# ayushpradhan-dev/robust-speech-analysis-framework

Measured on AMD Instinct MI355X. Metric: audio-seconds processed/sec (extract+CNN-LSTM fwd), higher is better.
Workload: dtype f32

## Files before the change

robust_speech_analysis_framework_amd/csrc/mshds_pitch.hip:

```cpp
#include <algorithm>
#include <map>
#include <mutex>
#include <vector>

#include "mshds_common.h"
#include "mshds_pitch_layout.h"

namespace rsaf {
namespace mshds {

struct PitchParams {
    double dt, min_pitch, ceiling, voicing_thr, octave_cost, dt_window;
    int cheb_all_full;
    int cheb_clipped;
    int nsamp_window, half_window, nsamp_period, half_period, min_lag, max_lag, brent_ixmax, max_cand;
    int refine_depth, is_cc;
    int nfft;
    double voicing_thr2;
    int debug_stop;
};

struct FrameOut {
    double intensity;
    double ncand;
// ... 593 lines not shown
            if (l0 + 1 <= L) {
                const double den = sumx2 * yb[m];
                rb[l0 + 1] = (l0 + 1 <= loc_max_lag && den > 0.0) ? (-y[m].y * inv_n) * fast_rsqrt(den) : 0.0;
            }
        }
        wave_sync();
    }
}

constexpr int CT = 64;
struct DeferArgs {
    FrameHdr* hdr;
    double* pc_a;
    double* pc_b;
    int grouped;
};
struct CandCtx {
    const PitchParams& P;
    const DeferArgs& DA;
    const double* cheb;
    int lane;
    int L, RC, RN;
    int nz_lo, nz_hi;
    double* r;
    double *s_mfreq, *s_mstr, *s_mloc;
    int* s_maxlag;
    int* s_cnt;
    double* s_part;
};

// ... 137 lines not shown
    const bool cand_lane = lane >= 1 && lane < nc;
    const int my_b0 = (cand_lane ? place_lag[lane] : 0) + RC - 1;
    if (use_cheb && !P.cheb_all_full) {
        int dc0 = P.refine_depth, dc1 = P.refine_depth;
        dc0 = dc0 < my_b0 + 1 ? dc0 : my_b0 + 1;
        dc0 = dc0 < RN - my_b0 - 1 ? dc0 : RN - my_b0 - 1;
        dc1 = dc1 < my_b0 + 2 ? dc1 : my_b0 + 2;
        dc1 = dc1 < RN - my_b0 - 2 ? dc1 : RN - my_b0 - 2;
        n_clip_cols = __popcll(__ballot(cand_lane && dc0 < P.refine_depth)) + __popcll(__ballot(cand_lane && dc1 < P.refine_depth));
        const int dmin = cand_row_min(cand_lane ? min(dc0, dc1) : P.refine_depth);
        if (n_clip_cols > 0 && (!P.cheb_clipped || dmin < 3)) use_cheb = false;
    }
    return CandClip{use_cheb, n_clip_cols, cand_lane, my_b0};
}

__device__ __forceinline__ void cand_coef_4x4x4(const CandCtx& X, int nc, const int* place_lag, const CandClip& C) {
    const double* cheb = X.cheb;
    const int lane = X.lane, RC = X.RC, nz_lo = X.nz_lo, nz_hi = X.nz_hi;
    const double* r = X.r;
    const bool cand_lane = C.cand_lane;
    const int my_b0 = C.my_b0;
    double* s_P = X.s_part;
    const int d = X.P.refine_depth;
    const int kq = lane >> 4, nn = lane & 15;
    const int ncol = 2 * (nc - 1);
    const int bmin = cand_row_min(cand_lane ? my_b0 : 0x7fffffff), bmax = -cand_row_min(cand_lane ? -my_b0 : 0x7fffffff);
    const int groups = (ncol + 3) >> 2;
    int rb4[3];
    bool cf4[3];
#pragma unroll
    for (int g = 0; g < 3; ++g) {
        const int n = 4 * g + (lane & 3), k = 1 + (n >> 1);
        rb4[g] = place_lag[k < nc ? k : 1] + RC - 1 + (n & 1);
        cf4[g] = n < ncol;
    }
    int o_lo = nz_lo - (bmax + 1), o_hi = nz_hi - bmin;
    o_lo = o_lo < -(d - 1) ? -(d - 1) : o_lo;
    o_hi = o_hi > d ? d : o_hi;
    double a4[3] = {0.0, 0.0, 0.0};
    const double* ctab = cheb + (int64_t)(d - 1) * NCH + nn;
    int o = o_lo;
    for (; o + 31 <= o_hi; o += 32) {
        double cw[8];
#pragma unroll
        for (int u = 0; u < 8; ++u) cw[u] = ctab[(int64_t)(o + 4 * u + kq) * NCH];
#pragma unroll
        for (int u = 0; u < 8; ++u) {
            const int oo = o + 4 * u + kq;
            a4[0] = __builtin_amdgcn_mfma_f64_4x4x4f64(cw[u], cf4[0] ? r[rb4[0] + oo] : 0.0, a4[0], 0, 0, 0);
            if (groups > 1) a4[1] = __builtin_amdgcn_mfma_f64_4x4x4f64(cw[u], cf4[1] ? r[rb4[1] + oo] : 0.0, a4[1], 0, 0, 0);
            if (groups > 2) a4[2] = __builtin_amdgcn_mfma_f64_4x4x4f64(cw[u], cf4[2] ? r[rb4[2] + oo] : 0.0, a4[2], 0, 0, 0);
        }
    }
    for (; o <= o_hi; o += 4) {
        const int oo = o + kq, oc = oo <= o_hi ? oo : o_hi;
        const double cw = oo <= o_hi ? ctab[(int64_t)oc * NCH] : 0.0;
        a4[0] = __builtin_amdgcn_mfma_f64_4x4x4f64(cw, cf4[0] ? r[rb4[0] + oc] : 0.0, a4[0], 0, 0, 0);
        if (groups > 1) a4[1] = __builtin_amdgcn_mfma_f64_4x4x4f64(cw, cf4[1] ? r[rb4[1] + oc] : 0.0, a4[1], 0, 0, 0);
        if (groups > 2) a4[2] = __builtin_amdgcn_mfma_f64_4x4x4f64(cw, cf4[2] ? r[rb4[2] + oc] : 0.0, a4[2], 0, 0, 0);
    }
    const int coef = (nn & 12) + kq;
#pragma unroll
    for (int g = 0; g < 3; ++g) {
        const int n = 4 * g + (lane & 3), k = 1 + (n >> 1);
        if (g < groups && n < ncol) s_P[(k * 2 + (n & 1)) * NCH + coef] = a4[g];
    }
}

__device__ __forceinline__ void cand_coef_16x16x4(const CandCtx& X, int nc, const int* place_lag, const CandClip& C) {
    const double* cheb = X.cheb;
    const int lane = X.lane, RC = X.RC, RN = X.RN, nz_lo = X.nz_lo, nz_hi = X.nz_hi;
    const double* r = X.r;
    const bool cand_lane = C.cand_lane;
    const int my_b0 = C.my_b0, n_clip_cols = C.n_clip_cols;
    double* s_P = X.s_part;
    const int d = X.P.refine_depth;
    const int kq = lane >> 4, nn = lane & 15;
    const int ncol = 2 * (nc - 1), tiles = (ncol + 15) >> 4;
    const int bmin = cand_row_min(cand_lane ? my_b0 : 0x7fffffff), bmax = -cand_row_min(cand_lane ? -my_b0 : 0x7fffffff);
    int rbase[2];
    bool colfull[2];
#pragma unroll
    for (int T = 0; T < 2; ++T) {
        const int n = 16 * T + nn, k = 1 + (n >> 1);
        rbase[T] = place_lag[k < nc ? k : 1] + RC - 1 + (n & 1);
        colfull[T] = n_clip_cols == 0 || (rbase[T] + 1 >= d && RN - rbase[T] - 1 >= d);
    }
    int o_lo = nz_lo - (bmax + 1), o_hi = nz_hi - bmin;
    o_lo = o_lo < -(d - 1) ? -(d - 1) : o_lo;
    o_hi = o_hi > d ? d : o_hi;
    double4_t acc0 = {0.0, 0.0, 0.0, 0.0}, acc1 = acc0;
    const double* ctab = cheb + (int64_t)(d - 1) * NCH + nn;
    int o = o_lo;
    for (; o + 31 <= o_hi; o += 32) {
        double cw[8];
#pragma unroll
        for (int u = 0; u < 8; ++u) cw[u] = ctab[(int64_t)(o + 4 * u + kq) * NCH];
#pragma unroll
        for (int u = 0; u < 8; ++u) {
            const int oo = o + 4 * u + kq;
            acc0 = __builtin_amdgcn_mfma_f64_16x16x4f64(cw[u], colfull[0] ? r[rbase[0] + oo] : 0.0, acc0, 0, 0, 0);
            if (tiles > 1) acc1 = __builtin_amdgcn_mfma_f64_16x16x4f64(cw[u], colfull[1] ? r[rbase[1] + oo] : 0.0, acc1, 0, 0, 0);
        }
    }
    for (; o <= o_hi; o += 4) {
        const int oo = o + kq, oc = oo <= o_hi ? oo : o_hi;
        const double cw = oo <= o_hi ? ctab[(int64_t)oc * NCH] : 0.0;
        acc0 = __builtin_amdgcn_mfma_f64_16x16x4f64(cw, colfull[0] ? r[rbase[0] + oc] : 0.0, acc0, 0, 0, 0);
        if (tiles > 1) acc1 = __builtin_amdgcn_mfma_f64_16x16x4f64(cw, colfull[1] ? r[rbase[1] + oc] : 0.0, acc1, 0, 0, 0);
    }
#pragma unroll
    for (int T = 0; T < 2; ++T) {
        const int n = 16 * T + nn, k = 1 + (n >> 1);
        if (T < tiles && k < nc) {
#pragma unroll
            for (int v = 0; v < 4; ++v) s_P[(k * 2 + (n & 1)) * NCH + kq + 4 * v] = T == 0 ? acc0[v] : acc1[v];
        }
    }
}

__device__ __forceinline__ void cand_coef_clipped_cells(const CandCtx& X, int nc, const int* place_lag) {
    const double* cheb = X.cheb;
    const int lane = X.lane, RC = X.RC, RN = X.RN;
    const double* r = X.r;
    double* s_P = X.s_part;
    const int d = X.P.refine_depth;
    const int ncol = 2 * (nc - 1);
    __builtin_amdgcn_fence(__ATOMIC_RELEASE, "workgroup");
    __builtin_amdgcn_wave_barrier();
    __builtin_amdgcn_fence(__ATOMIC_ACQUIRE, "workgroup");
    const double* clip_tabs = cheb + (int64_t)2 * d * NCH;
    const int jj = lane & 15, ph = lane >> 4;
    for (int col = 0; col < ncol; ++col) {
        const int k = 1 + (col >> 1), b = place_lag[k] + RC - 1 + (col & 1);
        int dc = d;
        dc = dc < b + 1 ? dc : b + 1;
        dc = dc < RN - b - 1 ? dc : RN - b - 1;
        if (dc >= d) continue;
        const double* tab = clip_tabs + (int64_t)NCH * dc * (dc - 1) + jj;
        double acc = 0.0;
        int o = -(dc - 1) + ph;
        for (; o + 12 <= dc; o += 16) {
            double tw4[4];
#pragma unroll
            for (int u = 0; u < 4; ++u) tw4[u] = tab[(int64_t)(o + 4 * u + dc - 1) * NCH];
#pragma unroll
            for (int u = 0; u < 4; ++u) acc = fma(tw4[u], r[b + o + 4 * u], acc);
        }
        for (; o <= dc; o += 4) acc = fma(tab[(int64_t)(o + dc - 1) * NCH], r[b + o], acc);
        acc += __shfl_xor(acc, 16, 64);
        acc += __shfl_xor(acc, 32, 64);
        if (ph == 0) s_P[(k * 2 + (col & 1)) * NCH + jj] = acc;
    }
}

__device__ __forceinline__ bool cand_hand_over_or_brent(const CandCtx& X, int nc, const int* place_lag, double* cf, double* cs,
                                                        double* pc_out) {
    const DeferArgs& DA = X.DA;
    const int tid = X.lane, RC = X.RC;
    const double* s_P = X.s_part;
    if (DA.hdr) {
        for (int i = 2 * NCH + tid; i < nc * 2 * NCH; i += CT) pc_out[i] = s_P[i];
        __syncthreads();
        return true;
    }
    if (tid < 64) {
        const int k = 1 + tid;
// ... 12 lines not shown
const int tid = X.lane, L = X.L, RC = X.RC, RN = X.RN, nz_lo = X.nz_lo, nz_hi = X.nz_hi;
const double* r = X.r;
    const int nref = nc - 1;
    const int span = P.refine_depth < 2 * L ? P.refine_depth : 2 * L;
    RefineArgs A{r, RN, RC, P.refine_depth, nz_lo, nz_hi, nc, place_lag, cf, cs};
    if (nref <= 4) { if (span >= 6 * 64) refine_candidates<64, true>(A, tid, CT); else refine_candidates<64, false>(A, tid, CT); }
    else if (nref <= 8) { if (span >= 6 * 32) refine_candidates<32, true>(A, tid, CT); else refine_candidates<32, false>(A, tid, CT); }
    else { if (span >= 6 * 16) refine_candidates<16, true>(A, tid, CT); else refine_candidates<16, false>(A, tid, CT); }
    __syncthreads();
}

__device__ __forceinline__ bool cand_refine_list(const CandCtx& X, int nc, const int* place_lag, double* cf, double* cs,
                                                 double* pc_out) {
    if (X.DA.hdr && X.DA.grouped) return true;
    const CandClip C = cand_clip_analysis(X, nc, place_lag);
    if (C.use_cheb) {
        const int ncol = 2 * (nc - 1);
        if (nc > 1 && ncol <= 12 && C.n_clip_cols == 0) {
            cand_coef_4x4x4(X, nc, place_lag, C);
        } else if (nc > 1) {
            cand_coef_16x16x4(X, nc, place_lag, C);
            if (C.n_clip_cols > 0) cand_coef_clipped_cells(X, nc, place_lag);
        }
        __syncthreads();
        if (X.P.debug_stop == 6) return true;
        return cand_hand_over_or_brent(X, nc, place_lag, cf, cs, pc_out);
    }
    cand_refine_direct(X, nc, place_lag, cf, cs);
    return false;
}

__device__ __forceinline__ void cand_write_hdr(FrameHdr* hdr, int tid, int flags, int n_a, const int* pl_a, int n_b,
                                               const int* pl_b, int hit) {
    if (tid < MAXC) {
        hdr->lag_a[tid] = (uint16_t)pl_a[tid];
        if (pl_b) {
            hdr->lag_b[tid] = (uint16_t)pl_b[tid];
// ... 18 lines not shown

__global__ __launch_bounds__(64) void pitch_cand_kernel(const ClipInfo* __restrict__ ci, const double* __restrict__ gpeak,
                                                        const PitchParams P, const double* __restrict__ rbuf, int rstride,
                                                        int max_frames, FrameOut* __restrict__ out,
                                                        FrameOut* __restrict__ out2, const double* __restrict__ cheb,
                                                        const DeferArgs DA) {
    extern __shared__ __attribute__((aligned(16))) char smem_raw[];
    const ClipInfo c = ci[blockIdx.y];
    const int f = blockIdx.x;
    if (f >= c.n_frames) return;
    const int tid = threadIdx.x, lane = tid & 63;
    const int L = P.is_cc ? P.max_lag : P.brent_ixmax;
    const int RC = P.brent_ixmax;
    const int RN = 2 * P.brent_ixmax + 1;
    int r_lo, r_hi;
    pitch_r_range(RC, L, P.min_lag, P.max_lag, (DA.hdr && DA.grouped) ? 30 : P.refine_depth, &r_lo, &r_hi);
    const CandLds lds(r_lo, r_hi);
    double* r_store = lds.r_store(smem_raw);
    double* r = r_store - (RC + r_lo);
    double* lists = lds.lists(smem_raw);
    int* ilists = reinterpret_cast<int*>(lists);
    double* s_mfreq = lists + CandLds::MFREQ;
    double* s_mstr = lists + CandLds::MSTR;
    double* s_mloc = lists + CandLds::MLOC;
    double* s_cf = lists + CandLds::CF;
    double* s_cs = lists + CandLds::CS;
    double* s_cloc = lists + CandLds::CLOC;
    int* s_maxlag = ilists + CandLds::MAXLAG;
    int* s_place = ilists + CandLds::PLACE;
    int* s_place2 = ilists + CandLds::PLACE2;
    int* s_cnt = ilists + CandLds::CNT;
// ... 182 lines not shown
        if (m1) qb[count + __popcll(b1 & below)] = ((unsigned)g << 5) | ((unsigned)m1 << 1) | 1u;
        count += __popcll(b1);
        wave_sync();
        int done = 0;
        for (; count - done >= 16; done += 16) run_tile(done, 16);
        const int left = count - done;
        const unsigned rest = lane < left ? qb[done + lane] : 0u;
        wave_sync();
        if (lane < left) qb[lane] = rest;
        count = left;
        wave_sync();
    }
    if (count > 0) run_tile(0, count);
}

__global__ __launch_bounds__(64) void pitch_brent_kernel(const ClipInfo* __restrict__ ci, const int* __restrict__ hdr,
                                                         const double* __restrict__ pc_a, const double* __restrict__ pc_b,
                                                         int max_frames, int RC, FrameOut* __restrict__ out_a,
                                                         FrameOut* __restrict__ out_b) {
    const ClipInfo c = ci[blockIdx.y];
    const int f0 = blockIdx.x * BR_FRAMES;
    if (f0 >= c.n_frames) return;
    const int lane = threadIdx.x;
    const int64_t g0 = (int64_t)blockIdx.y * max_frames + f0;
    int cnt_a = 0, cnt_b = 0;
    if (lane < BR_FRAMES && f0 + lane < c.n_frames) {
        const FrameHdr* h = FrameHdr::at(hdr, g0 + lane);
        const int flags = h->flags;
        if (flags & HDR_A_DEFER) cnt_a = h->n_a > 1 ? h->n_a - 1 : 0;
        if (flags & HDR_B_DEFER) cnt_b = h->n_b > 1 ? h->n_b - 1 : 0;
// ... 305 lines not shown
    FrameOut* frame_out;
    unsigned char* psi;
    int* end_state;
    double *sel_freq, *sel_strength, *stats;
    bool complete() const { return frame_out && psi && end_state && sel_freq && sel_strength && stats; }
};

struct PitchPlan {
    PitchParams P;
    double silence_thr, octave_jump, vuv;
    bool dual;
    int seg_len, Lr, rstride;
    int ncc, log2m, log2n;
    int wave_r;
    size_t lds_corr, lds_cand, lds_cell;
    int cell_b_lo, cell_n_b, cell_ntap_pad;
    bool defer;
    bool grouped;
    const double* cheb;
    int group;
    double corr_flops, corr_lds;
};

static int64_t cell_workgroups(const PitchPlan& pl, int64_t gframes, int* n_chunks_out) {
    const int64_t n_chunks = (gframes + CELL_CHUNK_FRAMES - 1) / CELL_CHUNK_FRAMES;
    if (n_chunks_out) *n_chunks_out = (int)n_chunks;
    return 8 * (int64_t)pl.cell_n_b * ((n_chunks + 7) / 8);
}

static int pitch_plan(const PitchCall& c, const double* h, const PitchOutputs& o1, const PitchOutputs& o2,
                      double voicing_thr2, PitchPlan* plan) {
    PitchPlan& pl = *plan;
    PitchParams& P = pl.P;
// ... 22 lines not shown
    RSAF_CHECK_ARG((P.is_cc ? P.max_lag : P.brent_ixmax) <= 1023, "more than 1023 lags (pitch floor below ~16 Hz) is not supported");
    P.nfft = 1;
    while ((double)P.nfft < (double)P.nsamp_window * 1.5) P.nfft *= 2;
    if (P.nfft < 16) P.nfft = 16;
    RSAF_CHECK_ARG(P.is_cc || P.nsamp_window + P.brent_ixmax <= P.nfft, "brent_ixmax must not exceed half the analysis window");
    const int seg_len = pl.seg_len = P.is_cc ? P.nsamp_window + P.max_lag + 1 : P.nsamp_window;
    const int Lr = pl.Lr = pitch_row_lags(h);
    pl.rstride = Lr + 2;
    int ncc = 64;
    while (ncc < seg_len) ncc *= 2;
    RSAF_CHECK_ARG(!P.is_cc || ncc <= 4096, "cross-correlation window + lag range longer than 4 095 samples is not supported");
    RSAF_CHECK_ARG(P.is_cc || P.nfft <= 4096, "autocorrelation window longer than 2 730 samples is not supported");
    pl.lds_corr = P.is_cc ? CcLds(ncc, Lr).bytes() : 0;
    pl.defer = getenv("RSAF_PITCH_INKERNEL") == nullptr;
    pl.grouped = pl.defer && table_mode == 2 && !dual && P.is_cc && c.sinc_cheb != nullptr;
    int r_lo_h, r_hi_h;
    pitch_r_range(P.brent_ixmax, Lr, P.min_lag, P.max_lag, pl.grouped ? 30 : P.refine_depth, &r_lo_h, &r_hi_h);
    pl.lds_cand = CandLds(r_lo_h, r_hi_h).bytes();
    RSAF_CHECK_ARG(pl.lds_corr <= 150 * 1024 && pl.lds_cand <= 150 * 1024, "analysis window too long for LDS");
    const int64_t row_bytes_per_clip = (int64_t)max_frames * PitchWs::bytes_per_frame(pl.rstride);
    RSAF_CHECK_ARG(max_frames == 0 || (c.workspace && c.workspace_bytes >= row_bytes_per_clip),
                   "workspace too small (rsaf_mshds_pitch_workspace_bytes)");
    int group = max_frames == 0 ? n_clips : (int)std::min<int64_t>(n_clips, c.workspace_bytes / std::max<int64_t>(row_bytes_per_clip, 1));
    if (max_frames > 0) group = (int)std::min<int64_t>(group, ((int64_t)1 << 26) / max_frames > 0 ? ((int64_t)1 << 26) / max_frames : 1);
    pl.group = group;
    RSAF_CHECK_ARG(table_mode != 2 || (!dual && P.is_cc), "per-cell tables serve single-threshold cross-correlation analyses only");
    pl.log2m = 0;
    while ((2 << pl.log2m) < P.nfft) ++pl.log2m;
    pl.log2n = 0;
    while ((1 << pl.log2n) < ncc) ++pl.log2n;
    int wave_r = 0;
    if (!P.is_cc) wave_r = pl.log2m <= 9 ? 8 : 1 << (pl.log2m - 6);
    else if (pl.log2n <= 11) wave_r = pl.log2n <= 10 ? 16 : 32;
    if (wave_r && !P.is_cc) P.nfft = 128 * wave_r;
    if (wave_r && P.is_cc) ncc = 64 * wave_r;
    pl.wave_r = wave_r;
    pl.ncc = ncc;
    pl.cheb = table_mode == 2 ? nullptr : c.sinc_cheb;
    const int cell_lag_lo = P.min_lag > 2 ? P.min_lag : 2;
    const int cell_lag_hi = std::min(P.max_lag - 1, P.brent_ixmax - 1);
    const bool unclipped = P.brent_ixmax + cell_lag_lo - 1 >= P.refine_depth && cell_lag_hi + 2 + P.refine_depth <= P.brent_ixmax;
    P.cheb_all_full = unclipped ? 1 : 0;
    if (pl.cheb == nullptr) P.cheb_clipped = 0;
    if (!unclipped && !P.cheb_clipped) pl.cheb = nullptr;
    pl.cell_b_lo = P.brent_ixmax + cell_lag_lo - 1;
    pl.cell_n_b = cell_lag_hi - cell_lag_lo + 2;
    pl.cell_ntap_pad = (Lr + 1 + 3) & ~3;
    pl.lds_cell = CellLds(pl.cell_ntap_pad).bytes();
    if (pl.grouped) {
        RSAF_CHECK_ARG(pl.cell_n_b >= 1 && pl.lds_cell <= 150 * 1024, "per-cell tables: lag range too long for LDS");
        if (max_frames > 0 && P.debug_stop == 0)
            RSAF_CHECK_ARG(cell_workgroups(pl, (int64_t)group * max_frames, nullptr) <= 0x7fffffffLL,
                           "per-cell tables: too many workgroups");
    }
    const double Mfft = 0.5 * (double)P.nfft;
    const double ac_flops = 2.0 * 5.0 * Mfft * log2(Mfft) + 30.0 * Mfft;
    const double cc_flops = 5.0 * ncc * log2((double)ncc) + 2.5 * ncc * log2(0.5 * ncc) + 40.0 * 0.5 * ncc + 4.0 * seg_len;
    const double ac_lds = 160.0 * Mfft;
    const double cc_lds = wave_r ? 120.0 * ncc + 16.0 * Lr
// ... 6 lines not shown
static int pitch_prepare(const PitchPlan& pl, const double2_t** tw_out, const double2_t** tw2_out) {
    if (!pl.wave_r)
        RSAF_CHECK_HIP(hipFuncSetAttribute((const void*)pitch_cc_kernel<12>, hipFuncAttributeMaxDynamicSharedMemorySize, (int)pl.lds_corr));
    const double *tw = nullptr, *tw2 = nullptr;
    int rc = fft_twiddles(pl.P.is_cc ? 2 * pl.ncc : pl.P.nfft, &tw);
    if (rc == RSAF_OK && pl.P.is_cc) rc = fft_twiddles(pl.ncc, &tw2);
    if (rc != RSAF_OK) return rc;
    *tw_out = reinterpret_cast<const double2_t*>(tw);
    *tw2_out = reinterpret_cast<const double2_t*>(tw2);
    if (pl.lds_cand > 48 * 1024)
        RSAF_CHECK_HIP(hipFuncSetAttribute((const void*)pitch_cand_kernel, hipFuncAttributeMaxDynamicSharedMemorySize,
                                           (int)pl.lds_cand));
    if (pl.grouped && pl.lds_cell > 48 * 1024)
        RSAF_CHECK_HIP(hipFuncSetAttribute((const void*)pitch_cell_coef_kernel, hipFuncAttributeMaxDynamicSharedMemorySize,
                                           (int)pl.lds_cell));
    return RSAF_OK;
}

struct PitchGroup {
    const ClipInfo* ci;
    const double* gpeak;
    int nc;
    PitchWs ws;
};

static PitchGroup pitch_group(const PitchCall& c, const PitchPlan& pl, int c0) {
    const int nc = std::min(pl.group, c.n_clips - c0);
    return PitchGroup{c.ci + c0, c.gpeak + c0, nc, PitchWs(c.workspace, (int64_t)nc * c.max_frames, pl.rstride)};
}

// ... 21 lines not shown
            case 16: launch_cc_wave<16>(c, pl, g, wave_grid, tw2); break;
            case 32: launch_cc_wave<32>(c, pl, g, wave_grid, tw2); break;
        }
    else
        switch (pl.wave_r) {
            case 8: launch_ac_wave<8>(c, pl, g, wave_grid, tw); break;
            case 16: launch_ac_wave<16>(c, pl, g, wave_grid, tw); break;
            case 32: launch_ac_wave<32>(c, pl, g, wave_grid, tw); break;
        }
    RSAF_CHECK_HIP(hipGetLastError());
    return RSAF_OK;
}

static int launch_candidates(const PitchCall& c, const PitchPlan& pl, const PitchGroup& g, FrameOut* out, FrameOut* out2) {
    const double rows = (double)c.max_frames * (double)g.nc;
    const DeferArgs DA{pl.defer ? g.ws.hdr : nullptr, pl.defer ? g.ws.pc_a : nullptr, pl.defer ? g.ws.pc_b : nullptr, pl.grouped ? 1 : 0};
    ProfScope prof(pl.grouped ? "mshds_pitch_cand_lists" : pl.cheb ? "mshds_pitch_cand_cheb" : "mshds_pitch_cand_direct", c.stream,
                   pl.cheb ? rows * 2048.0 * 2.0 * ceil(2.0 * pl.P.refine_depth / 4.0) : 0.0,
                   rows * (double)(pl.Lr + 2) * 8.0);
    hipLaunchKernelGGL(pitch_cand_kernel, dim3(c.max_frames, g.nc), dim3(CT), pl.lds_cand, c.stream, g.ci, g.gpeak, pl.P,
                       (const double*)g.ws.rows, pl.rstride, c.max_frames, out, out2, pl.cheb, DA);
    RSAF_CHECK_HIP(hipGetLastError());
    return RSAF_OK;
}

static int launch_refinement(const PitchCall& c, const PitchPlan& pl, const PitchGroup& g, FrameOut* out, FrameOut* out2) {
    const double rows = (double)c.max_frames * (double)g.nc;
    if (pl.grouped) {
        int n_chunks;
        const int64_t n_wg = cell_workgroups(pl, (int64_t)g.nc * c.max_frames, &n_chunks);
        ProfScope prof("mshds_pitch_cand_cells", c.stream, rows * 28.0 * 2.0 * pl.cell_ntap_pad * NCH,
                       rows * 28.0 * (double)(pl.Lr + 1) * 8.0);
        hipLaunchKernelGGL(pitch_cell_coef_kernel, dim3((unsigned)n_wg), dim3(256), pl.lds_cell, c.stream, g.ci, g.nc, c.max_frames,
                           (const int*)g.ws.hdr, (const double*)g.ws.rows, pl.rstride, pl.Lr, pl.P.brent_ixmax, c.sinc_cheb,
                           pl.cell_b_lo, pl.cell_n_b, pl.cell_ntap_pad, CELL_CHUNK_FRAMES, n_chunks, g.ws.pc_a);
        RSAF_CHECK_HIP(hipGetLastError());
    }
    const bool low_is_second = pl.dual && pl.P.voicing_thr2 < pl.P.voicing_thr;
    FrameOut* oa = low_is_second ? out2 : out;
    FrameOut* ob = low_is_second ? out : out2;
    ProfScope prof("mshds_pitch_cand_brent", c.stream, 0.0, rows * 15.0 * 2.0 * NCH * 8.0);
    hipLaunchKernelGGL(pitch_brent_kernel, dim3((c.max_frames + BR_FRAMES - 1) / BR_FRAMES, g.nc), dim3(64), 0, c.stream, g.ci,
                       (const int*)g.ws.hdr, (const double*)g.ws.pc_a, (const double*)g.ws.pc_b, c.max_frames, pl.P.brent_ixmax, oa, ob);
    RSAF_CHECK_HIP(hipGetLastError());
    return RSAF_OK;
}

static int launch_paths(const PitchCall& c, const PitchPlan& pl, const PitchOutputs& o, double voicing_thr) {
    const PitchParams& P = pl.P;
    {
// ... 66 lines not shown
```

robust_speech_analysis_framework_amd/csrc/mshds_pitch_layout.h:

```cpp
#pragma once
#include <cstddef>
#include <cstdint>

#if defined(__HIPCC__)
#define PL_HD __host__ __device__ __forceinline__
#else
#define PL_HD inline
#endif

namespace rsaf {
namespace mshds {

constexpr int MAXC = 16;
constexpr int MAX_MAXIMA = 96;
constexpr int NCH = 16;
constexpr int PC_DOUBLES = MAXC * 2 * NCH;
constexpr int CELL_Q = 192;
constexpr int WF_FRAMES = 8;
constexpr int CC_FRAMES_PER_WG = 16;
constexpr int BR_FRAMES = 16;
constexpr int CELL_CHUNK_FRAMES = 4096;

PL_HD void pitch_r_range(int rc, int L, int min_lag, int max_lag, int depth, int* lo, int* hi) {
    const int w = 2 * L + 2, span = w < rc ? w : rc;
    const int lag_lo = min_lag > 2 ? min_lag : 2;
    int lag_hi = max_lag - 1;
    if (lag_hi > rc - 1) lag_hi = rc - 1;
    const int d = depth > 30 ? depth : 30;
    int a = lag_lo - d - 3, b = lag_hi + d + 3;
    *lo = a < -span ? -span : a;
    *hi = b > span ? span : b;
}

constexpr int HDR_A_DEFER = 1, HDR_B_DEFER = 2, HDR_B_COPY = 4;
struct FrameHdr {
    int flags;
    int n_a, n_b;
    int unused0;
    uint16_t lag_a[MAXC];
    uint16_t lag_b[MAXC];
    uint8_t a_slot_of_b[MAXC];
    uint8_t unused1[32];
    PL_HD uint32_t lag_a_pair(int i) const { return reinterpret_cast<const uint32_t*>(lag_a)[i]; }
    PL_HD uint32_t a_slot_of_b_quad(int i) const { return reinterpret_cast<const uint32_t*>(a_slot_of_b)[i]; }
    static PL_HD const FrameHdr* at(const int* records, int64_t frame);
};
static_assert(sizeof(FrameHdr) == 128, "one 128-byte record per frame");
// ... 45 lines not shown
    int fft_doubles, sy_doubles;
    PL_HD CcWaveLds(int plan_doubles, int L) : fft_doubles(plan_doubles), sy_doubles((L + 3) & ~1) {}
    PL_HD double* fft(char* lds) const { return reinterpret_cast<double*>(lds); }
    PL_HD double* sy(char* lds) const { return fft(lds) + fft_doubles; }
    PL_HD size_t bytes() const { return (size_t)(fft_doubles + sy_doubles) * sizeof(double); }
};

struct CellLds {
    int tab_doubles;
    PL_HD explicit CellLds(int ntap_pad) : tab_doubles(ntap_pad * NCH) {}
    PL_HD double* tab(char* lds) const { return reinterpret_cast<double*>(lds); }
    PL_HD unsigned* queues(char* lds) const { return reinterpret_cast<unsigned*>(tab(lds) + tab_doubles); }
    PL_HD size_t bytes() const { return (size_t)tab_doubles * sizeof(double) + 4 * CELL_Q * sizeof(unsigned); }
};

struct PitchWs {
    double* rows;
    double *pc_a, *pc_b;
    FrameHdr* hdr;
    static PL_HD int64_t bytes_per_frame(int rstride) {
        return (int64_t)rstride * (int64_t)sizeof(double) + 2 * (int64_t)PC_DOUBLES * (int64_t)sizeof(double) + (int64_t)sizeof(FrameHdr);
    }
    PL_HD PitchWs(double* workspace, int64_t frames, int rstride) {
        rows = workspace;
        pc_a = rows + frames * rstride;
        pc_b = pc_a + frames * PC_DOUBLES;
        hdr = reinterpret_cast<FrameHdr*>(pc_b + frames * PC_DOUBLES);
    }
};

// ... 3 lines not shown
```

robust_speech_analysis_framework_amd/mshds.py:

```python
from __future__ import annotations

import collections
import ctypes as C
import math
import os

import numpy as np

from . import _lib
from .wavio import read_wav_mono_device

FS = 16000.0
DX = 1.0 / FS
SAMPLE_RATE = 16000

FEATURE_NAMES = [
    "Speaking_Rate", "Articulation_Rate", "Phonation_Ratio", "Pause_Rate", "Mean_Pause_Duration",
    "mean_F0", "stdev_F0_Semitone", "mean_dB", "range_ratio_dB", "HNR_dB",
    "Spectral_Slope", "Spectral_Tilt", "Cepstral_Peak_Prominence",
    "mean_F1_Loc", "std_F1_Loc", "mean_B1_Loc", "std_B1_Loc",
    "mean_F2_Loc", "std_F2_Loc", "mean_B2_Loc", "std_B2_Loc",
    "Spectral_Gravity", "Spectral_Std_Dev", "Spectral_Skewness", "Spectral_Kurtosis",
]
BUILT_COLUMNS = [0, 1, 2, 3, 4, 5, 6, 7, 8, 9, 10, 11, 12, 13, 14, 15, 16, 17, 18, 19, 20, 21, 22, 23, 24]
# ... 199 lines not shown
def lowpass_eligible(lengths):
    cap = int(_lib.load().rsaf_praat_lowpass_max_samples())
    return [int(n) <= cap for n in lengths]


class MshdsEngine:
    def __init__(self, device="cuda"):
        import torch
        _lib.load()
        _lib.require_gpu()
        self.device = torch.device(device)
        self._tables = {}
        self.fo_doubles = _lib.load().rsaf_mshds_frameout_doubles()
        self.n_streams = 3
        self._aux = None

    def _table(self, key, builder):
        if key not in self._tables:
            self._tables[key] = tuple(None if a is None else _dev(np.asarray(a, dtype=np.float64), self.device, blocking=True)
                                      for a in builder())
        return self._tables[key]

    def _pitch_outputs(self, tf, n):
        import torch
        dev = self.device
        return {"frame_out": torch.empty(tf * self.fo_doubles, dtype=torch.float64, device=dev),
                "psi": torch.empty(tf * 16, dtype=torch.uint8, device=dev),
                "end_state": torch.empty(max(n, 1), dtype=torch.int32, device=dev),
                "sel_freq": torch.zeros(tf, dtype=torch.float64, device=dev),
                "sel_strength": torch.zeros(tf, dtype=torch.float64, device=dev),
# ... 25 lines not shown
                                   octave_jump_cost, voiced_unvoiced_cost, g.nsamp_window, g.nsamp_period, g.min_lag,
                                   g.max_lag, g.brent_ixmax, max_candidates, refine_depth, 1 if is_cc else 0,
                                   g.dt_window, table_mode)
        second = None
        if voicing_threshold2 is not None:
            second = {"geom": g, "ci": ci, "ci_dev": ci_d, "total_frames": total, "max_frames": mx, **self._pitch_outputs(tf, n)}
        wp = _lib.ptr(win) if win is not None else None
        wrp = _lib.ptr(wr) if wr is not None else None
        if cheb is None:
            (cheb,) = self._table(("sinc_cheb", int(refine_depth), clipped_tables),
                                  lambda: (sinc_cheb_tables(int(refine_depth), clipped_tables),))
        chp = _lib.ptr(cheb)
        per_clip = int(lib.rsaf_mshds_pitch_workspace_bytes_per_clip(mx, params)) if n else 0
        ws_bytes = max(per_clip * max(1, min(n, int(self.pitch_ws_cap_bytes // max(per_clip, 1)))), 8)
        ws = torch.empty(ws_bytes // 8, dtype=torch.float64, device=dev)
        def ptrs(o):
            return [_lib.ptr(o[k]) for k in first]
        if n and g.half_window >= 2:
            if second is None:
                _lib.check(lib.rsaf_mshds_pitch(
                    _lib.ptr(wav), _lib.ptr(ci_d), n, mx, _lib.ptr(gpeak), wp, wrp, params, *ptrs(first),
                    chp, _lib.ptr(ws), ws_bytes, _lib.stream_ptr(stream)), "rsaf_mshds_pitch")
            else:
                _lib.check(lib.rsaf_mshds_pitch_dual(
                    _lib.ptr(wav), _lib.ptr(ci_d), n, mx, _lib.ptr(gpeak), wp, wrp, params, *ptrs(first),
                    float(voicing_threshold2), *ptrs(second), chp, _lib.ptr(ws), ws_bytes, _lib.stream_ptr(stream)),
                    "rsaf_mshds_pitch_dual")
        else:
            for o in (first, second) if second is not None else (first,):
                o["stats"].fill_(float("nan"))
# ... 430 lines not shown
```

Baseline: 12430.

## Move unclipped sinc-Chebyshev coefficient MFMA into a separate shared-table kernel

Adds a deferred kernel that stages the Chebyshev table in LDS and batches candidate columns from many frames into 16-wide MFMA tiles. The per-frame candidate kernel now skips this work in shared mode and computes only the clipped cells. The change also removes the 4x4x4 MFMA path and aligns the 16x16x4 tap loop to a 4-aligned grid with masking. It aims to raise MFMA utilization and table reuse, at the cost of an extra launch, more global traffic for window gathers, and a wider r-range LDS footprint in the all-full case.

```diff
diff --git a/robust_speech_analysis_framework_amd/csrc/mshds_pitch.hip b/robust_speech_analysis_framework_amd/csrc/mshds_pitch.hip
--- a/robust_speech_analysis_framework_amd/csrc/mshds_pitch.hip
+++ b/robust_speech_analysis_framework_amd/csrc/mshds_pitch.hip
@@ -631,6 +631,7 @@
     double* pc_a;
     double* pc_b;
     int grouped;
+    int shared;
 };
 struct CandCtx {
     const PitchParams& P;
@@ -798,59 +799,6 @@
     return CandClip{use_cheb, n_clip_cols, cand_lane, my_b0};
 }
 
-__device__ __forceinline__ void cand_coef_4x4x4(const CandCtx& X, int nc, const int* place_lag, const CandClip& C) {
-    const double* cheb = X.cheb;
-    const int lane = X.lane, RC = X.RC, nz_lo = X.nz_lo, nz_hi = X.nz_hi;
-    const double* r = X.r;
-    const bool cand_lane = C.cand_lane;
-    const int my_b0 = C.my_b0;
-    double* s_P = X.s_part;
-    const int d = X.P.refine_depth;
-    const int kq = lane >> 4, nn = lane & 15;
-    const int ncol = 2 * (nc - 1);
-    const int bmin = cand_row_min(cand_lane ? my_b0 : 0x7fffffff), bmax = -cand_row_min(cand_lane ? -my_b0 : 0x7fffffff);
-    const int groups = (ncol + 3) >> 2;
-    int rb4[3];
-    bool cf4[3];
-#pragma unroll
-    for (int g = 0; g < 3; ++g) {
-        const int n = 4 * g + (lane & 3), k = 1 + (n >> 1);
-        rb4[g] = place_lag[k < nc ? k : 1] + RC - 1 + (n & 1);
-        cf4[g] = n < ncol;
-    }
-    int o_lo = nz_lo - (bmax + 1), o_hi = nz_hi - bmin;
-    o_lo = o_lo < -(d - 1) ? -(d - 1) : o_lo;
-    o_hi = o_hi > d ? d : o_hi;
-    double a4[3] = {0.0, 0.0, 0.0};
-    const double* ctab = cheb + (int64_t)(d - 1) * NCH + nn;
-    int o = o_lo;
-    for (; o + 31 <= o_hi; o += 32) {
-        double cw[8];
-#pragma unroll
-        for (int u = 0; u < 8; ++u) cw[u] = ctab[(int64_t)(o + 4 * u + kq) * NCH];
-#pragma unroll
-        for (int u = 0; u < 8; ++u) {
-            const int oo = o + 4 * u + kq;
-            a4[0] = __builtin_amdgcn_mfma_f64_4x4x4f64(cw[u], cf4[0] ? r[rb4[0] + oo] : 0.0, a4[0], 0, 0, 0);
-            if (groups > 1) a4[1] = __builtin_amdgcn_mfma_f64_4x4x4f64(cw[u], cf4[1] ? r[rb4[1] + oo] : 0.0, a4[1], 0, 0, 0);
-            if (groups > 2) a4[2] = __builtin_amdgcn_mfma_f64_4x4x4f64(cw[u], cf4[2] ? r[rb4[2] + oo] : 0.0, a4[2], 0, 0, 0);
-        }
-    }
-    for (; o <= o_hi; o += 4) {
-        const int oo = o + kq, oc = oo <= o_hi ? oo : o_hi;
-        const double cw = oo <= o_hi ? ctab[(int64_t)oc * NCH] : 0.0;
-        a4[0] = __builtin_amdgcn_mfma_f64_4x4x4f64(cw, cf4[0] ? r[rb4[0] + oc] : 0.0, a4[0], 0, 0, 0);
-        if (groups > 1) a4[1] = __builtin_amdgcn_mfma_f64_4x4x4f64(cw, cf4[1] ? r[rb4[1] + oc] : 0.0, a4[1], 0, 0, 0);
-        if (groups > 2) a4[2] = __builtin_amdgcn_mfma_f64_4x4x4f64(cw, cf4[2] ? r[rb4[2] + oc] : 0.0, a4[2], 0, 0, 0);
-    }
-    const int coef = (nn & 12) + kq;
-#pragma unroll
-    for (int g = 0; g < 3; ++g) {
-        const int n = 4 * g + (lane & 3), k = 1 + (n >> 1);
-        if (g < groups && n < ncol) s_P[(k * 2 + (n & 1)) * NCH + coef] = a4[g];
-    }
-}
-
 __device__ __forceinline__ void cand_coef_16x16x4(const CandCtx& X, int nc, const int* place_lag, const CandClip& C) {
     const double* cheb = X.cheb;
     const int lane = X.lane, RC = X.RC, RN = X.RN, nz_lo = X.nz_lo, nz_hi = X.nz_hi;
@@ -873,25 +821,27 @@
     int o_lo = nz_lo - (bmax + 1), o_hi = nz_hi - bmin;
     o_lo = o_lo < -(d - 1) ? -(d - 1) : o_lo;
     o_hi = o_hi > d ? d : o_hi;
+    int g_lo, g_hi;
+    pitch_tap_grid(d, o_lo, o_hi, &g_lo, &g_hi);
     double4_t acc0 = {0.0, 0.0, 0.0, 0.0}, acc1 = acc0;
     const double* ctab = cheb + (int64_t)(d - 1) * NCH + nn;
-    int o = o_lo;
-    for (; o + 31 <= o_hi; o += 32) {
+    for (int o = g_lo; o <= g_hi; o += 32) {
         double cw[8];
-#pragma unroll
-        for (int u = 0; u < 8; ++u) cw[u] = ctab[(int64_t)(o + 4 * u + kq) * NCH];
+        bool in[8];
 #pragma unroll
         for (int u = 0; u < 8; ++u) {
             const int oo = o + 4 * u + kq;
-            acc0 = __builtin_amdgcn_mfma_f64_16x16x4f64(cw[u], colfull[0] ? r[rbase[0] + oo] : 0.0, acc0, 0, 0, 0);
-            if (tiles > 1) acc1 = __builtin_amdgcn_mfma_f64_16x16x4f64(cw[u], colfull[1] ? r[rbase[1] + oo] : 0.0, acc1, 0, 0, 0);
-        }
-    }
-    for (; o <= o_hi; o += 4) {
-        const int oo = o + kq, oc = oo <= o_hi ? oo : o_hi;
-        const double cw = oo <= o_hi ? ctab[(int64_t)oc * NCH] : 0.0;
-        acc0 = __builtin_amdgcn_mfma_f64_16x16x4f64(cw, colfull[0] ? r[rbase[0] + oc] : 0.0, acc0, 0, 0, 0);
-        if (tiles > 1) acc1 = __builtin_amdgcn_mfma_f64_16x16x4f64(cw, colfull[1] ? r[rbase[1] + oc] : 0.0, acc1, 0, 0, 0);
+            in[u] = oo >= o_lo && oo <= o_hi;
+            cw[u] = ctab[(int64_t)(in[u] ? oo : o_lo) * NCH];
+        }
+#pragma unroll
+        for (int u = 0; u < 8; ++u) {
+            if (o + 4 * u > g_hi) break;
+            const int oc = in[u] ? o + 4 * u + kq : o_lo;
+            acc0 = __builtin_amdgcn_mfma_f64_16x16x4f64(in[u] ? cw[u] : 0.0, in[u] && colfull[0] ? r[rbase[0] + oc] : 0.0, acc0, 0, 0, 0);
+            if (tiles > 1)
+                acc1 = __builtin_amdgcn_mfma_f64_16x16x4f64(in[u] ? cw[u] : 0.0, in[u] && colfull[1] ? r[rbase[1] + oc] : 0.0, acc1, 0, 0, 0);
+        }
     }
 #pragma unroll
     for (int T = 0; T < 2; ++T) {
@@ -903,11 +853,10 @@
     }
 }
 
-__device__ __forceinline__ void cand_coef_clipped_cells(const CandCtx& X, int nc, const int* place_lag) {
+__device__ __forceinline__ void cand_coef_clipped_cells(const CandCtx& X, int nc, const int* place_lag, double* dst) {
     const double* cheb = X.cheb;
     const int lane = X.lane, RC = X.RC, RN = X.RN;
     const double* r = X.r;
-    double* s_P = X.s_part;
     const int d = X.P.refine_depth;
     const int ncol = 2 * (nc - 1);
     __builtin_amdgcn_fence(__ATOMIC_RELEASE, "workgroup");
@@ -934,7 +883,7 @@
         for (; o <= dc; o += 4) acc = fma(tab[(int64_t)(o + dc - 1) * NCH], r[b + o], acc);
         acc += __shfl_xor(acc, 16, 64);
         acc += __shfl_xor(acc, 32, 64);
-        if (ph == 0) s_P[(k * 2 + (col & 1)) * NCH + jj] = acc;
+        if (ph == 0) dst[(k * 2 + (col & 1)) * NCH + jj] = acc;
     }
 }
 
@@ -977,13 +926,14 @@
                                                  double* pc_out) {
     if (X.DA.hdr && X.DA.grouped) return true;
     const CandClip C = cand_clip_analysis(X, nc, place_lag);
+    if (C.use_cheb && X.DA.hdr && X.DA.shared) {
+        if (nc > 1 && C.n_clip_cols > 0) cand_coef_clipped_cells(X, nc, place_lag, pc_out);
+        return true;
+    }
     if (C.use_cheb) {
-        const int ncol = 2 * (nc - 1);
-        if (nc > 1 && ncol <= 12 && C.n_clip_cols == 0) {
-            cand_coef_4x4x4(X, nc, place_lag, C);
-        } else if (nc > 1) {
+        if (nc > 1) {
             cand_coef_16x16x4(X, nc, place_lag, C);
-            if (C.n_clip_cols > 0) cand_coef_clipped_cells(X, nc, place_lag);
+            if (C.n_clip_cols > 0) cand_coef_clipped_cells(X, nc, place_lag, X.s_part);
         }
         __syncthreads();
         if (X.P.debug_stop == 6) return true;
@@ -1032,7 +982,8 @@
     const int RC = P.brent_ixmax;
     const int RN = 2 * P.brent_ixmax + 1;
     int r_lo, r_hi;
-    pitch_r_range(RC, L, P.min_lag, P.max_lag, (DA.hdr && DA.grouped) ? 30 : P.refine_depth, &r_lo, &r_hi);
+    pitch_r_range(RC, L, P.min_lag, P.max_lag, cand_reach_depth(P.refine_depth, DA.hdr && DA.grouped, DA.hdr && DA.shared && P.cheb_all_full),
+                  &r_lo, &r_hi);
     const CandLds lds(r_lo, r_hi);
     double* r_store = lds.r_store(smem_raw);
     double* r = r_store - (RC + r_lo);
@@ -1245,6 +1196,171 @@
     if (count > 0) run_tile(0, count);
 }
 
+__global__ __launch_bounds__(256, 2) void pitch_shared_coef_kernel(const ClipInfo* __restrict__ ci, int n_clips, int max_frames,
+                                                                const int* __restrict__ hdr, const double* __restrict__ rbuf,
+                                                                int rstride, int L, int RC, int d, int all_full,
+                                                                const double* __restrict__ cheb, double* __restrict__ pc_a,
+                                                                double* __restrict__ pc_b) {
+    using namespace wfft;
+    extern __shared__ __attribute__((aligned(16))) char smem_raw[];
+    const SharedLds lds(d);
+    double* tab = lds.tab(smem_raw);
+    const int tid = threadIdx.x, lane = tid & 63, wv = tid >> 6;
+    const int nn = lane & 15, kq = lane >> 4;
+    const int wstride = lds.win_stride;
+    const double* zero = lds.zero(smem_raw);
+    if (tid == 0) lds.zero(smem_raw)[0] = 0.0;
+    double* win = lds.windows(smem_raw) + wv * SharedLds::WINDOWS * wstride;
+    const int RN = 2 * RC + 1, nz_lo = RC - L, nz_hi = RC + L;
+    const int64_t total = (int64_t)n_clips * max_frames;
+    constexpr int per_wave = SHARED_CHUNK_FRAMES / 4;
+    const int64_t g_begin = (int64_t)blockIdx.x * SHARED_CHUNK_FRAMES + (int64_t)wv * per_wave;
+    const int64_t g_end = g_begin + per_wave < total ? g_begin + per_wave : total;
+    auto load_counts = [&](int64_t g, int& ca, int& cb) {
+        ca = cb = 0;
+        if (g < g_end) {
+            const int clip = (int)(g / max_frames), fr = (int)(g - (int64_t)clip * max_frames);
+            if (fr < ci[clip].n_frames) {
+                const FrameHdr* h = FrameHdr::at(hdr, g);
+                const int flags = h->flags, n_a = h->n_a, n_b = h->n_b;
+                if ((flags & HDR_A_DEFER) && n_a > 1 && n_a < MAXC) ca = 2 * (n_a - 1);
+                if ((flags & HDR_B_DEFER) && n_b > 1 && n_b < MAXC) cb = 2 * (n_b - 1);
+            }
+        }
+    };
+    int ca, cb;
+    load_counts(g_begin + lane, ca, cb);
+    {
+        const int n_tab = 2 * d * NCH, n_all = lds.tab_doubles;
+        const double2_t* src = reinterpret_cast<const double2_t*>(cheb);
+        double2_t* dst = reinterpret_cast<double2_t*>(tab);
+        const int n2 = n_tab / 2, m2 = n_all / 2;
+        for (int i0 = tid; i0 < m2; i0 += 8 * 256) {
+            double2_t v[8];
+#pragma unroll
+            for (int u = 0; u < 8; ++u) v[u] = src[i0 + 256 * u < n2 ? i0 + 256 * u : n2 - 1];
+#pragma unroll
+            for (int u = 0; u < 8; ++u)
+                if (i0 + 256 * u < m2) dst[i0 + 256 * u] = i0 + 256 * u < n2 ? v[u] : double2_t{0.0, 0.0};
+        }
+    }
+    __syncthreads();
+    for (int64_t g0 = g_begin; g0 < g_end; g0 += 64) {
+        const int tot = ca + cb;
+        int incl = tot;
+#pragma unroll
+        for (int o = 1; o < 64; o <<= 1) { const int up = __shfl_up(incl, o, 64); if (lane >= o) incl += up; }
+        const int excl = incl - tot;
+        const int T = __builtin_amdgcn_readlane(incl, 63);
+        const int ca_now = ca;
+        if (T == 0) { load_counts(g0 + 64 + lane, ca, cb); continue; }
+        load_counts(g0 + 64 + lane, ca, cb);
+        struct Col { int j, k, cell, lag; bool is_b, valid; };
+        auto column = [&](int t0) {
+            const bool valid = t0 + nn < T;
+            const int q = valid ? t0 + nn : (t0 < T ? t0 : 0);
+            int j = 0;
+#pragma unroll
+            for (int s = 32; s >= 1; s >>= 1) { if (__shfl(incl, j + s - 1, 64) <= q) j += s; }
+            j &= 63;
+            const int rr = q - __shfl(excl, j, 64), na = __shfl(ca_now, j, 64);
+            Col c;
+            c.is_b = rr >= na;
+            const int idx = c.is_b ? rr - na : rr;
+            c.k = 1 + (idx >> 1);
+            c.cell = idx & 1;
+            c.j = g0 + j < g_end ? j : 0;
+            const FrameHdr* h = FrameHdr::at(hdr, g0 + c.j);
+            c.lag = (int)(c.is_b ? h->lag_b : h->lag_a)[c.k];
+            c.valid = valid;
+            return c;
+        };
+        auto left_sample = [&](const Col& c) { return c.lag + RC - 1 + c.cell; };
+        double wreg[8][3];
+        auto win_load = [&](const Col& c, int t0) {
+#pragma unroll
+            for (int w = 0; w < 8; ++w) {
+                if (t0 + 2 * w >= T) break;
+                const int b0 = __builtin_amdgcn_readlane(left_sample(c), 2 * w), jw = __builtin_amdgcn_readlane(c.j, 2 * w);
+                const double* rb = rbuf + (g0 + jw) * rstride;
+#pragma unroll
+                for (int u = 0; u < 3; ++u) {
+                    const int lg = b0 - (d - 1) + lane + 64 * u - RC, l = lg < 0 ? -lg : lg;
+                    wreg[w][u] = rb[l <= L ? l : L];
+                }
+            }
+        };
+        auto win_store = [&](const Col& c, int t0) {
+#pragma unroll
+            for (int w = 0; w < 8; ++w) {
+                if (t0 + 2 * w >= T) break;
+                const int b0 = __builtin_amdgcn_readlane(left_sample(c), 2 * w);
+#pragma unroll
+                for (int u = 0; u < 3; ++u) {
+                    const int i = lane + 64 * u, lg = b0 - (d - 1) + i - RC, l = lg < 0 ? -lg : lg;
+                    if (i < wstride) win[w * wstride + i] = l <= L ? wreg[w][u] : 0.0;
+                }
+            }
+        };
+        Col cur = column(0), ahead = column(16);
+        win_load(cur, 0);
+        for (int t0 = 0; t0 < T; t0 += 16) {
+            win_store(cur, t0);
+            wave_sync();
+            const Col c = cur;
+            cur = ahead;
+            if (t0 + 16 < T) win_load(cur, t0 + 16);
+            ahead = column(t0 + 32);
+            const int b = left_sample(c);
+            const bool on = c.valid && (all_full || (b + 1 >= d && RN - b - 1 >= d));
+            const int bmin = cand_row_min(on ? b : 0x7fffffff), bmax = -cand_row_min(on ? -b : 0x7fffffff);
+            if (bmin != 0x7fffffff) {
+                int o_lo = nz_lo - bmax, o_hi = nz_hi - bmin;
+                o_lo = o_lo < -(d - 1) ? -(d - 1) : o_lo;
+                o_hi = o_hi > d ? d : o_hi;
+                int g_lo, g_hi;
+                pitch_tap_grid(d, o_lo, o_hi, &g_lo, &g_hi);
+                const int ntap = g_hi - g_lo + 1;
+                const double* wcol = win + (nn >> 1) * wstride + (nn & 1) + (d - 1);
+                const double* tcol = tab + (d - 1) * NCH + nn;
+                double4_t acc = {0.0, 0.0, 0.0, 0.0};
+                double av[2][8], bv[2][8];
+                auto fetch = [&](int tb, double (&a8)[8], double (&b8)[8]) {
+#pragma unroll
+                    for (int u = 0; u < 8; ++u) {
+                        const int t = tb + 4 * u + kq;
+                        const int o = g_lo + (t < ntap ? t : 0);
+                        a8[u] = tcol[o * NCH];
+                        b8[u] = *((on && o <= d) ? wcol + o : zero);
+                    }
+                };
+                fetch(0, av[0], bv[0]);
+                for (int tb = 0; tb < ntap; tb += 64) {
+                    if (tb + 32 < ntap) fetch(tb + 32, av[1], bv[1]);
+#pragma unroll
+                    for (int u = 0; u < 8; ++u) {
+                        if (tb + 4 * u >= ntap) break;
+                        acc = __builtin_amdgcn_mfma_f64_16x16x4f64(av[0][u], bv[0][u], acc, 0, 0, 0);
+                    }
+                    if (tb + 32 >= ntap) break;
+                    if (tb + 64 < ntap) fetch(tb + 64, av[0], bv[0]);
+#pragma unroll
+                    for (int u = 0; u < 8; ++u) {
+                        if (tb + 32 + 4 * u >= ntap) break;
+                        acc = __builtin_amdgcn_mfma_f64_16x16x4f64(av[1][u], bv[1][u], acc, 0, 0, 0);
+                    }
+                }
+                if (on) {
+                    double* dst = (c.is_b ? pc_b : pc_a) + ((g0 + c.j) * MAXC + c.k) * (2 * NCH) + c.cell * NCH;
+#pragma unroll
+                    for (int v = 0; v < 4; ++v) dst[kq + 4 * v] = acc[v];
+                }
+            }
+            wave_sync();
+        }
+    }
+}
+
 __global__ __launch_bounds__(64) void pitch_brent_kernel(const ClipInfo* __restrict__ ci, const int* __restrict__ hdr,
                                                          const double* __restrict__ pc_a, const double* __restrict__ pc_b,
                                                          int max_frames, int RC, FrameOut* __restrict__ out_a,
@@ -1580,9 +1696,11 @@
     int ncc, log2m, log2n;
     int wave_r;
     size_t lds_corr, lds_cand, lds_cell;
+    size_t lds_shared;
     int cell_b_lo, cell_n_b, cell_ntap_pad;
     bool defer;
     bool grouped;
+    bool shared;
     const double* cheb;
     int group;
     double corr_flops, corr_lds;
@@ -1635,10 +1753,7 @@
     pl.lds_corr = P.is_cc ? CcLds(ncc, Lr).bytes() : 0;
     pl.defer = getenv("RSAF_PITCH_INKERNEL") == nullptr;
     pl.grouped = pl.defer && table_mode == 2 && !dual && P.is_cc && c.sinc_cheb != nullptr;
-    int r_lo_h, r_hi_h;
-    pitch_r_range(P.brent_ixmax, Lr, P.min_lag, P.max_lag, pl.grouped ? 30 : P.refine_depth, &r_lo_h, &r_hi_h);
-    pl.lds_cand = CandLds(r_lo_h, r_hi_h).bytes();
-    RSAF_CHECK_ARG(pl.lds_corr <= 150 * 1024 && pl.lds_cand <= 150 * 1024, "analysis window too long for LDS");
+    RSAF_CHECK_ARG(pl.lds_corr <= 150 * 1024, "analysis window too long for LDS");
     const int64_t row_bytes_per_clip = (int64_t)max_frames * PitchWs::bytes_per_frame(pl.rstride);
     RSAF_CHECK_ARG(max_frames == 0 || (c.workspace && c.workspace_bytes >= row_bytes_per_clip),
                    "workspace too small (rsaf_mshds_pitch_workspace_bytes)");
@@ -1664,6 +1779,13 @@
     P.cheb_all_full = unclipped ? 1 : 0;
     if (pl.cheb == nullptr) P.cheb_clipped = 0;
     if (!unclipped && !P.cheb_clipped) pl.cheb = nullptr;
+    pl.lds_shared = SharedLds(P.refine_depth).bytes();
+    pl.shared = pl.defer && !pl.grouped && pl.cheb != nullptr && P.refine_depth >= 1 && SharedLds(P.refine_depth).fits();
+    int r_lo_h, r_hi_h;
+    pitch_r_range(P.brent_ixmax, Lr, P.min_lag, P.max_lag,
+                  cand_reach_depth(P.refine_depth, pl.grouped, pl.shared && P.cheb_all_full), &r_lo_h, &r_hi_h);
+    pl.lds_cand = CandLds(r_lo_h, r_hi_h).bytes();
+    RSAF_CHECK_ARG(pl.lds_cand <= 150 * 1024, "analysis window too long for LDS");
     pl.cell_b_lo = P.brent_ixmax + cell_lag_lo - 1;
     pl.cell_n_b = cell_lag_hi - cell_lag_lo + 2;
     pl.cell_ntap_pad = (Lr + 1 + 3) & ~3;
@@ -1700,6 +1822,9 @@
     if (pl.grouped && pl.lds_cell > 48 * 1024)
         RSAF_CHECK_HIP(hipFuncSetAttribute((const void*)pitch_cell_coef_kernel, hipFuncAttributeMaxDynamicSharedMemorySize,
                                            (int)pl.lds_cell));
+    if (pl.shared && pl.lds_shared > 48 * 1024)
+        RSAF_CHECK_HIP(hipFuncSetAttribute((const void*)pitch_shared_coef_kernel, hipFuncAttributeMaxDynamicSharedMemorySize,
+                                           (int)pl.lds_shared));
     return RSAF_OK;
 }
 
@@ -1751,7 +1876,8 @@
 
 static int launch_candidates(const PitchCall& c, const PitchPlan& pl, const PitchGroup& g, FrameOut* out, FrameOut* out2) {
     const double rows = (double)c.max_frames * (double)g.nc;
-    const DeferArgs DA{pl.defer ? g.ws.hdr : nullptr, pl.defer ? g.ws.pc_a : nullptr, pl.defer ? g.ws.pc_b : nullptr, pl.grouped ? 1 : 0};
+    const DeferArgs DA{pl.defer ? g.ws.hdr : nullptr, pl.defer ? g.ws.pc_a : nullptr, pl.defer ? g.ws.pc_b : nullptr, pl.grouped ? 1 : 0,
+                       pl.shared ? 1 : 0};
     ProfScope prof(pl.grouped ? "mshds_pitch_cand_lists" : pl.cheb ? "mshds_pitch_cand_cheb" : "mshds_pitch_cand_direct", c.stream,
                    pl.cheb ? rows * 2048.0 * 2.0 * ceil(2.0 * pl.P.refine_depth / 4.0) : 0.0,
                    rows * (double)(pl.Lr + 2) * 8.0);
@@ -1771,6 +1897,16 @@
         hipLaunchKernelGGL(pitch_cell_coef_kernel, dim3((unsigned)n_wg), dim3(256), pl.lds_cell, c.stream, g.ci, g.nc, c.max_frames,
                            (const int*)g.ws.hdr, (const double*)g.ws.rows, pl.rstride, pl.Lr, pl.P.brent_ixmax, c.sinc_cheb,
                            pl.cell_b_lo, pl.cell_n_b, pl.cell_ntap_pad, CELL_CHUNK_FRAMES, n_chunks, g.ws.pc_a);
+        RSAF_CHECK_HIP(hipGetLastError());
+    }
+    if (pl.shared) {
+        const int64_t gframes = (int64_t)g.nc * c.max_frames;
+        ProfScope prof("mshds_pitch_cand_shared", c.stream, rows * 6.0 * 2.0 * pitch_tap_rows(pl.P.refine_depth) * NCH,
+                       rows * 6.0 * 2.0 * pl.P.refine_depth * 8.0);
+        hipLaunchKernelGGL(pitch_shared_coef_kernel, dim3((unsigned)((gframes + SHARED_CHUNK_FRAMES - 1) / SHARED_CHUNK_FRAMES)),
+                           dim3(256), pl.lds_shared, c.stream, g.ci, g.nc, c.max_frames, (const int*)g.ws.hdr,
+                           (const double*)g.ws.rows, pl.rstride, pl.Lr, pl.P.brent_ixmax, pl.P.refine_depth, pl.P.cheb_all_full,
+                           pl.cheb, g.ws.pc_a, g.ws.pc_b);
         RSAF_CHECK_HIP(hipGetLastError());
     }
     const bool low_is_second = pl.dual && pl.P.voicing_thr2 < pl.P.voicing_thr;
diff --git a/robust_speech_analysis_framework_amd/csrc/mshds_pitch_layout.h b/robust_speech_analysis_framework_amd/csrc/mshds_pitch_layout.h
--- a/robust_speech_analysis_framework_amd/csrc/mshds_pitch_layout.h
+++ b/robust_speech_analysis_framework_amd/csrc/mshds_pitch_layout.h
@@ -20,6 +20,8 @@
 constexpr int CC_FRAMES_PER_WG = 16;
 constexpr int BR_FRAMES = 16;
 constexpr int CELL_CHUNK_FRAMES = 4096;
+constexpr int SHARED_CHUNK_FRAMES = 256;
+constexpr int SHARED_LDS_MAX = 64 * 1024;
 
 PL_HD void pitch_r_range(int rc, int L, int min_lag, int max_lag, int depth, int* lo, int* hi) {
     const int w = 2 * L + 2, span = w < rc ? w : rc;
@@ -31,6 +33,17 @@
     *lo = a < -span ? -span : a;
     *hi = b > span ? span : b;
 }
+
+PL_HD int cand_reach_depth(int refine_depth, bool per_cell, bool shared_all_full) {
+    return (per_cell || shared_all_full) ? 30 : refine_depth;
+}
+
+PL_HD void pitch_tap_grid(int d, int o_lo, int o_hi, int* g_lo, int* g_hi) {
+    const int first = -(d - 1);
+    *g_lo = first + ((o_lo - first) & ~3);
+    *g_hi = o_hi < o_lo ? *g_lo - 1 : first + ((o_hi - first) | 3);
+}
+PL_HD int pitch_tap_rows(int d) { return (2 * d + 3) & ~3; }
 
 constexpr int HDR_A_DEFER = 1, HDR_B_DEFER = 2, HDR_B_COPY = 4;
 struct FrameHdr {
@@ -106,6 +119,18 @@
     PL_HD size_t bytes() const { return (size_t)tab_doubles * sizeof(double) + 4 * CELL_Q * sizeof(unsigned); }
 };
 
+struct SharedLds {
+    static constexpr int WINDOWS = 8, WINDOW_MAX = 192;
+    int tab_doubles, win_stride;
+    PL_HD explicit SharedLds(int depth)
+        : tab_doubles(pitch_tap_rows(depth) * NCH), win_stride(((pitch_tap_rows(depth) + 31) & ~31) + 4) {}
+    PL_HD bool fits() const { return win_stride <= WINDOW_MAX && bytes() <= (size_t)SHARED_LDS_MAX; }
+    PL_HD double* tab(char* lds) const { return reinterpret_cast<double*>(lds); }
+    PL_HD double* windows(char* lds) const { return tab(lds) + tab_doubles; }
+    PL_HD double* zero(char* lds) const { return windows(lds) + 4 * WINDOWS * win_stride; }
+    PL_HD size_t bytes() const { return (size_t)(tab_doubles + 4 * WINDOWS * win_stride + 2) * sizeof(double); }
+};
+
 struct PitchWs {
     double* rows;
     double *pc_a, *pc_b;
diff --git a/robust_speech_analysis_framework_amd/mshds.py b/robust_speech_analysis_framework_amd/mshds.py
--- a/robust_speech_analysis_framework_amd/mshds.py
+++ b/robust_speech_analysis_framework_amd/mshds.py
@@ -237,6 +237,8 @@
         self.fo_doubles = _lib.load().rsaf_mshds_frameout_doubles()
         self.n_streams = 3
         self._aux = None
+        self.pitch_debug = None
+        self._last_pitch = None
 
     def _table(self, key, builder):
         if key not in self._tables:
@@ -292,6 +294,12 @@
         per_clip = int(lib.rsaf_mshds_pitch_workspace_bytes_per_clip(mx, params)) if n else 0
         ws_bytes = max(per_clip * max(1, min(n, int(self.pitch_ws_cap_bytes // max(per_clip, 1)))), 8)
         ws = torch.empty(ws_bytes // 8, dtype=torch.float64, device=dev)
+        if self.pitch_debug is not None:
+            if self.pitch_debug.get("fill") is not None:
+                ws.fill_(float(self.pitch_debug["fill"]))
+            group = max(1, min(n, ws_bytes // max(per_clip, 1)))
+            self._last_pitch = {"ws": ws, "group": group, "rstride": (g.max_lag if is_cc else g.brent_ixmax) + 2,
+                                "max_frames": mx, "table": cheb, "table_mode": table_mode}
         def ptrs(o):
             return [_lib.ptr(o[k]) for k in first]
         if n and g.half_window >= 2:
```

Result: no change. 12460 (median of 2 runs) (+0.3%).
